# dlwns147/amq

Measured on AMD Instinct MI355X. Metric: decode tokens/s, Llama-2-7B AMQ mixed 2/3/4-bit avg-3-bit, batch 1, higher is better.
Workload: dtype f16; 1 GPU; Llama-2-7B shapes, synthesized avg-3.0-bit per-layer arch (bits_usage 2.982), batch 1 decode after a 64-token prefill, one stream per GPU; parallelism=replicas x1, prompt=64, group_size=128

## Files before the change

amq_amd/_lib.py:

```python
import ctypes
import os

_HERE = os.path.dirname(os.path.abspath(__file__))
LIB_PATH = os.path.join(_HERE, "libamq_hip.so")
AB_LIB_PATH = os.path.join(_HERE, "libamq_hip_ab.so")

AMQ_OK = 0
MODE_HQQ, MODE_FMA, MODE_FMA1 = 0, 1, 2
PRO_NONE, PRO_RMSNORM, PRO_SILU_MUL = 0, 1, 2
MAX_SEGMENTS = 4
MATH_DEFAULT, MATH_LINEAR, MATH_GROUPSCALE, MATH_EXACT = 0, 1, 2, 3
FEWROW_AUTO, FEWROW_TILE, FEWROW_STREAM = 0, 1, 2
ABI_VERSION = 521
LOOKUP_STATE_WORDS = 32
STEP_STATE_STRIDE = 272
GEMM_AUTO, GEMM_TILED, GEMM_SKINNY, GEMM_RING, GEMM_RING128, GEMM_WS, GEMM_DEQ = 0, 1, 2, 3, 4, 5, 6

_vp, _i, _f, _sz = ctypes.c_void_p, ctypes.c_int, ctypes.c_float, ctypes.c_size_t


class Segment(ctypes.Structure):
    _fields_ = [("qweight_native", _vp), ("meta_native", _vp), ("bias", _vp), ("residual", _vp),
                ("y", _vp), ("N", _i), ("bits", _i), ("mode", _i), ("y_stride", _i)]

# ... 32 lines not shown
    "amq_gemm_f16": (_i, [_i, _i, _vp, _vp, _vp, _vp, _vp, _i, _i, _i, _i, _i, _i, _vp]),
    "amq_linear_f16": (_i, [_i, _i, _vp, _vp, _vp, _vp, _vp, _i, _i, _i, _i, _vp]),
    "amq_gemm_splitk_workspace_bytes": (_sz, [_i, _i, _i]),
    "amq_gemm_splitk_f16": (_i, [_i, _i, _vp, _vp, _vp, _vp, _vp, _i, _i, _i, _i, _i, _i, _vp, _sz, _vp]),
    "amq_compat_workspace_bytes": (_sz, [_i, _i, _i, _i]),
    "amq_vecquantmatmul_faster_old": (_i, [_i, _vp, _vp, _vp, _vp, _vp, _i, _i, _i, _i, _i, _vp, _sz, _i, _vp]),
    "amq_gemv_4bit": (_i, [_vp, _vp, _vp, _vp, _vp, _i, _i, _i, _i, _vp, _sz, _i, _vp]),
    "amq_gemm_4bit": (_i, [_vp, _vp, _vp, _vp, _vp, _i, _i, _i, _i, _vp, _sz, _i, _vp]),
    "amq_rmsnorm_f16": (_i, [_vp, _vp, _vp, _i, _i, _f, _vp]),
    "amq_gemv_f16w": (_i, [_vp, _vp, _vp, _vp, _vp, _f, _i, _i, _vp]),
    "amq_attn_decode_f16": (_i, [_vp, _vp, _vp, _vp, _vp, _vp, _vp, _i, _i, _i, _i, _i, _i, _f, _vp, _vp]),
    "amq_rope_table_f16": (_i, [_vp, _i, _f, _vp]),
    "amq_rope_table_freqs_f16": (_i, [_vp, _i, _vp, _f, _vp]),
    "amq_decode_tail_f16": (_i, [_vp, _i, _vp, _i, _vp, _vp, _vp, _vp, _vp, _i, _vp]),
    "amq_attn_decode_cur_f16": (_i, [_vp, _vp, _vp, _vp, _vp, _vp, _vp, _i, _i, _i, _i, _i, _vp]),
    "amq_gemm_res_f16": (_i, [_i, _i, _vp, _vp, _vp, _vp, _vp, _vp, _i, _i, _i, _i, _i, _i, _vp, _sz, _vp]),
    "amq_xfrag_bytes": (_sz, [_i, _i]),
    "amq_xfrag_f16": (_i, [_vp, _vp, _i, _i, ctypes.c_longlong, ctypes.c_longlong, _vp]),
    "amq_rmsnorm_xfrag_f16": (_i, [_vp, _vp, _vp, _i, _i, _f, _vp]),
    "amq_gemm_xfrag_f16": (_i, [_i, _i, _vp, _vp, _vp, _vp, _vp, _vp, _vp, _i, _i, _i, _i, _i, _vp]),
    "amq_gemm_gated_fused": (_i, [_i, _i, _i, _i, _i]),
    "amq_gemm_gated_fused_g": (_i, [_i, _i, _i, _i, _i, _i]),
    "amq_gemm_gated_f16": (_i, [_i, _i, _i, _vp, _vp, _vp, _vp, _vp, _vp, _i, _i, _i, _i, _i, _vp, _sz, _vp]),
    "amq_attn_decode_split_workspace_bytes": (_sz, [_i, _i, _i]),
    "amq_attn_decode_split_f16": (_i, [_vp, _vp, _vp, _vp, _vp, _vp, _vp, _vp, _i, _i, _i, _i, _i, _i, _f, _vp, _i, _vp, _sz, _vp, _vp]),
    "amq_gemm_xfrag_grouped_f16": (_i, [ctypes.POINTER(Segment), _i, _vp, _i, _i, _i, _vp]),
    "amq_gemm_xfrag_grouped_form_f16": (_i, [ctypes.POINTER(Segment), _i, _vp, _i, _i, _i, _i, _i, _vp]),
    "amq_attn_prefill_xfrag_f16": (_i, [_vp, _vp, _vp, _vp, _i, _i, _i, _i, _i] + [ctypes.c_longlong] * 5 + [_vp]),
    "amq_gemv_f16w_rows": (_i, [_vp, _vp, _vp, _vp, _vp, _f, _i, _i, _i, _vp]),
    "amq_decode_tail_batch_f16": (_i, [_vp, _i, _vp, _i, _vp, _vp, _vp, _vp, _vp, _i, _i, _vp]),
    "amq_decode_tail_suppress_f16": (_i, [_vp, _i, _vp, _i, _vp, _vp, _vp, _vp, _vp, _i, _i, _vp, _vp]),
    "amq_sample_f16": (_i, [_vp, _i, _i, _vp, _vp, _vp, _vp, _vp, _i, _i, _vp]),
    "amq_decode_tail_sample_f16": (_i, [_vp, _i, _vp, _i, _vp, _vp, _vp, _vp, _vp, _i, _i, _vp, _vp, _vp]),
    "amq_set_token_f16": (_i, [_vp, _i, _vp, _i, _i, _vp, _vp, _vp, _vp, _vp, _i, _i, _vp]),
    "amq_attn_decode_seq_f16": (_i, [_vp, _vp, _vp, _vp, _vp, _vp, _vp, _i, _i, _i, _i, _i, _i, _vp, _sz, _vp, _vp]),
    "amq_decode_tail_seq_f16": (_i, [_vp, _i, _vp, _i, _vp, _vp, _vp, _vp, _i, _i, _vp, _vp]),
    "amq_decode_tail_sample_seq_f16": (_i, [_vp, _i, _vp, _i, _vp, _vp, _vp, _vp, _i, _i, _vp, _vp, _vp]),
    "amq_set_token_seq_f16": (_i, [_vp, _i, _vp, _i, _i, _vp, _vp, _vp, _vp, _i, _i, _vp]),
    "amq_attn_decode_rows_f16": (_i, [_vp, _vp, _vp, _vp, _vp, _vp, _vp, _i, _i, _i, _i, _i, _i, _vp, _sz, _vp, _vp]),
    "amq_decode_tail_lookup_f16": (_i, [_vp, _i, _vp, _i, _vp, _vp, _vp, _vp, _i, _i, _vp, _vp, _vp, _i, _vp]),
    "amq_attn_prefill_f16": (_i, [_vp, _vp, _vp, _vp, _i, _i, _i, _i, _i, _i] + [ctypes.c_longlong] * 10 + [_vp]),
    "amq_rope_cache_f16": (_i, [_vp, _vp, _vp, _vp, _vp, _vp, _i, _i, _i, _i, _i, _i, _i, _vp]),
    "amq_rope_cache_batch_f16": (_i, [_vp, _vp, _vp, _vp, _vp, _vp, _i, _i, _i, _i, _i, _i, _i, _i, _vp]),
    "amq_rope_rows_f16": (_i, [_vp, _vp, _vp, _i, _i, _i, _i, _i, _i, _i, _vp]),
    "amq_silu_mul_f16": (_i, [_vp, _vp, _vp, _sz, _vp]),
    "amq_gemv_grouped_f16": (_i, [ctypes.POINTER(Segment), _i, _vp, _vp, _vp, _f, _i, _i, _i, _i, _i, ctypes.POINTER(GemvOpts), _vp]),
    "amq_gemv_grouped_sums_f16": (_i, [ctypes.POINTER(Segment), _i, _vp, _vp, _f, _vp, _vp, _i, _i, _i, _vp]),
    "amq_gemm_f16w_f16": (_i, [_vp, _vp, _vp, _vp, _vp, _vp, _i, _i, _i, _i, _i, _vp]),
    "amq_gemm_route_workspace_bytes": (_sz, [_i, _i, _i, _i]),
    "amq_gemm_route_workspace_bytes_g": (_sz, [_i, _i, _i, _i, _i]),
# ... 135 lines not shown
```

amq_amd/csrc/amq_capi.hip:

```cpp
#include "../../include/amq_hip.h"
#ifdef AMQ_AB_ROUTES
#include "../../include/amq_hip_ab.h"
#endif
#include "amq_common.cuh"
#include "amq_kernels.h"

#include <stdarg.h>
#include <stdio.h>
#include <vector>

namespace {

thread_local char g_err[512] = "";

int fail(int code, const char* fmt, ...) {
    va_list ap;
    va_start(ap, fmt);
    vsnprintf(g_err, sizeof(g_err), fmt, ap);
    va_end(ap);
    return code;
}

int check_hip(hipError_t e, const char* what) {
    if (e == hipSuccess) return AMQ_OK;
// ... 695 lines not shown

int amq_attn_decode_cur_f16(const void* q, const void* k, const void* v, void* kcache, void* vcache, void* out,
                            const void* step_state, int batch, int n_heads, int n_kv_heads, int head_dim, int max_seq,
                            void* stream) {
    if (!q || !k || !v || !kcache || !vcache || !out || !step_state) return fail(AMQ_EINVAL, "null pointer");
    if (n_heads > 255) return fail(AMQ_ESHAPE, "at most 255 heads");
    if (head_dim != 128) return fail(AMQ_ESHAPE, "head_dim must be 128 (got %d)", head_dim);
    if (batch < 1 || n_heads < 1 || n_kv_heads < 1 || (n_heads % n_kv_heads) != 0)
        return fail(AMQ_ESHAPE, "bad head configuration (%d q heads, %d kv heads)", n_heads, n_kv_heads);
    if (max_seq < 1) return fail(AMQ_ESHAPE, "bad max_seq %d", max_seq);
    if (6 * 128 + (size_t)max_seq * 4 + 17 * 1024 > LDS_LIMIT) return fail(AMQ_ESHAPE, "max_seq=%d too long for the single-pass decode attention", max_seq);
    amq::AttnArgs a{q, k, v, kcache, vcache, out, nullptr, 0, n_heads, n_kv_heads, max_seq, 10000.0f, nullptr, step_state};
    return check_hip(amq::launch_attn_decode(a, batch, (hipStream_t)stream), "attn_decode_cur");
}

size_t amq_attn_decode_split_workspace_bytes(int batch, int n_heads, int n_splits) {
    if (batch < 1 || n_heads < 1 || n_splits < 1) return 0;
    return (size_t)batch * n_heads * n_splits * 132 * sizeof(float);
}

int amq_attn_decode_split_f16(const void* q, const void* k, const void* v, void* kcache, void* vcache, void* out,
                              const void* step_state, const int* pos_dev, int pos, int batch, int n_heads, int n_kv_heads,
                              int head_dim, int max_seq, float rope_theta, const void* rope_table, int n_splits,
                              void* workspace, size_t workspace_bytes, void* tickets, void* stream) {
    if (!q || !k || !v || !kcache || !vcache || !out || !workspace || !tickets) return fail(AMQ_EINVAL, "null pointer");
    if (head_dim != 128) return fail(AMQ_ESHAPE, "head_dim must be 128 (got %d)", head_dim);
    if (batch < 1 || batch > 65535 || n_heads < 1 || n_heads > 255 || n_kv_heads < 1 || (n_heads % n_kv_heads) != 0)
        return fail(AMQ_ESHAPE, "bad head configuration (batch %d, %d q heads, %d kv heads)", batch, n_heads, n_kv_heads);
    if (n_splits < 1 || n_splits > 1024) return fail(AMQ_EINVAL, "n_splits must be 1..1024 (got %d)", n_splits);
    if (max_seq < 1 || (!step_state && !pos_dev && (pos < 0 || pos >= max_seq)))
// ... 135 lines not shown
    if (max_seq < 1) return fail(AMQ_ESHAPE, "bad max_seq %d", max_seq);
    if (n_splits < 0 || n_splits > 1024) return fail(AMQ_EINVAL, "n_splits must be 0 (one workgroup per head) or 1..1024 (got %d)", n_splits);
    amq::AttnArgs a{q, k, v, kcache, vcache, out, nullptr, 0, n_heads, n_kv_heads, max_seq, 10000.0f, nullptr, step_states, true};
    if (n_splits == 0) {
        if (6 * 128 + (size_t)max_seq * 4 + 17 * 1024 > LDS_LIMIT) return fail(AMQ_ESHAPE, "max_seq=%d too long for the single-pass decode attention", max_seq);
        return check_hip(amq::launch_attn_decode(a, batch, (hipStream_t)stream), "attn_decode_seq");
    }
    if (!workspace || !tickets) return fail(AMQ_EINVAL, "null pointer (workspace / tickets are required with n_splits >= 1)");
    int chunk = (((max_seq + n_splits - 1) / n_splits) + 31) & ~31;
    chunk = chunk < amq::ATT_MIN_CHUNK ? amq::ATT_MIN_CHUNK : chunk;
    if (6 * 128 + (size_t)chunk * 4 + 17 * 1024 > LDS_LIMIT)
        return fail(AMQ_ESHAPE, "max_seq=%d over %d splits leaves chunks of %d keys: too long", max_seq, n_splits, chunk);
    const size_t need = amq_attn_decode_split_workspace_bytes(batch, n_heads, n_splits);
    if (workspace_bytes < need) return fail(AMQ_EINVAL, "workspace too small: need %zu bytes, got %zu", need, workspace_bytes);
    return check_hip(amq::launch_attn_decode_split(a, batch, n_splits, workspace, tickets, (hipStream_t)stream), "attn_decode_seq (split)");
}

static int tail_seq_check(const void* logits, int vocab, const void* embed, int hidden, const void* token, const void* step_states, const void* x,
                          const void* rope_table, int rope_rows, int batch) {
    if (!logits || !embed || !token || !step_states || !x || !rope_table) return fail(AMQ_EINVAL, "null pointer");
    if (rope_rows < 1) return fail(AMQ_EINVAL, "rope_rows must be the number of rows of rope_table");
    if (vocab < 1 || hidden < 8 || (hidden % 8) != 0) return fail(AMQ_ESHAPE, "need vocab >= 1 and hidden %% 8 == 0 (got %d, %d)", vocab, hidden);
    if (batch < 1 || batch > 65535) return fail(AMQ_ESHAPE, "bad batch %d", batch);
    return AMQ_OK;
}

int amq_decode_tail_seq_f16(const void* logits, int vocab, const void* embed, int hidden, long long* token, void* step_states, void* x,
                            const void* rope_table, int rope_rows, int batch, const int* suppress_ids, void* stream) {
    if (int rc = tail_seq_check(logits, vocab, embed, hidden, token, step_states, x, rope_table, rope_rows, batch)) return rc;
    if (batch > 1 && (vocab % 8) != 0) return fail(AMQ_ESHAPE, "batched rows need vocab %% 8 == 0 (16-byte aligned logits rows)");
// ... 80 lines not shown
```

amq_amd/csrc/amq_decode.hip:

```cpp
#include "amq_common.cuh"
#include "amq_kernels.h"

namespace amq {

__device__ __forceinline__ float wave_sum_f(float v) {
#pragma unroll
    for (int off = 32; off > 0; off >>= 1) v += __shfl_xor(v, off);
    return v;
}
__device__ __forceinline__ float wave_max_f(float v) {
#pragma unroll
    for (int off = 32; off > 0; off >>= 1) v = fmaxf(v, __shfl_xor(v, off));
    return v;
}

template <bool FRAG>
__global__ __launch_bounds__(256) void rmsnorm_kernel(const _Float16* x, const _Float16* gamma, _Float16* y, int M, int K, float eps) {
    __shared__ float red[4];
    const int m = blockIdx.x;
    const bool live = m < M;
    const _Float16* xr = x + (size_t)(live ? m : 0) * K;
    float ss = 0.f;
    for (int c = threadIdx.x; c < (K >> 3); c += 256) {
        h8 v = *(const h8*)(xr + 8 * c);
// ... 299 lines not shown
                       __builtin_bit_cast(float, __builtin_amdgcn_readlane(__builtin_bit_cast(int, v), 16))),
                 fmaxf(__builtin_bit_cast(float, __builtin_amdgcn_readlane(__builtin_bit_cast(int, v), 32)),
                       __builtin_bit_cast(float, __builtin_amdgcn_readlane(__builtin_bit_cast(int, v), 48))));
}

constexpr int ATT_THREADS = 512;
constexpr int ATT_GROUPS = ATT_THREADS / 16;
constexpr int ATT_PF = 12;
#ifndef AMQ_ATT_SPEC
#define AMQ_ATT_SPEC 2
#endif
constexpr int ATT_SPEC = AMQ_ATT_SPEC;

struct AttnRest {
    void* out; const void* rope_table; int pos; float rope_theta;
#ifdef AMQ_STAMP
    unsigned long long* stamps;
#endif
};
#ifdef AMQ_STAMP
extern unsigned long long* g_stamp_ptr;
#define ATT_STAMP(slot_) do { if (rest.stamps && threadIdx.x == 0) rest.stamps[(size_t)blockIdx.x * 16 + (slot_)] = __builtin_amdgcn_s_memrealtime(); } while (0)
#else
#define ATT_STAMP(slot_) do { } while (0)
#endif

constexpr int ATT_ROWS_MAX = 8;
constexpr int ATT_ROWS_LDS = 2 * (ATT_ROWS_MAX - 1) * ATT_D * 2;
template <bool SEQ, bool ROWS = false>
__global__ __launch_bounds__(ATT_THREADS) void attn_decode_kernel(void* p_kc, void* p_vc, const void* p_state, int p_heads,
                                                                   int p_max_seq, const void* p_q, const void* p_k,
                                                                   const void* p_v, AttnRest rest) {
    const void* const p_state0 = p_state;
    if (SEQ) p_state = (const char*)p_state + (size_t)blockIdx.y * STEP_STRIDE;
    extern __shared__ __attribute__((aligned(16))) unsigned char smem[];
    _Float16* qs = (_Float16*)smem;
    _Float16* ks = (_Float16*)smem + ATT_D;
    _Float16* vs = (_Float16*)smem + 2 * ATT_D;
    float* sc = (float*)(smem + 6 * ATT_D);
    __shared__ float red[2 * ATT_THREADS / 64];
    __shared__ float part[ATT_GROUPS][ATT_D];
    const int h = blockIdx.x, b = blockIdx.y, tid = threadIdx.x;
    const int cb = ROWS ? 0 : b;
    const int n_heads = p_heads & 0xFF, n_kv_heads = (p_heads >> 8) & 0xFF, max_seq = p_max_seq;
    const bool cur_mode = (p_heads >> 16) & 1;
    const void* p_cur = cur_mode ? p_state : nullptr;
    int pos;
    if (cur_mode) pos = *(const int*)((const char*)p_state + 256);
    else if (p_state) pos = *(const int*)p_state;
    else pos = rest.pos;
    const int group = n_heads / n_kv_heads;
    const int kvh = h / group;
    const int grp = tid >> 4, l16 = tid & 15;
    const _Float16* q = (const _Float16*)p_q + ((size_t)b * n_heads + h) * ATT_D;
    const _Float16* kn = (const _Float16*)p_k + ((size_t)b * n_kv_heads + kvh) * ATT_D;
    const _Float16* vn = (const _Float16*)p_v + ((size_t)b * n_kv_heads + kvh) * ATT_D;
    _Float16* kc = (_Float16*)p_kc + ((size_t)cb * n_kv_heads + kvh) * (size_t)max_seq * ATT_D;
    _Float16* vc = (_Float16*)p_vc + ((size_t)cb * n_kv_heads + kvh) * (size_t)max_seq * ATT_D;

    ATT_STAMP(0);
    _Float16 q0 = 0, q1 = 0, k0 = 0, k1 = 0, v0 = 0, v1 = 0;
    h2 cs_cur = {(_Float16)1.f, (_Float16)0.f}, cs_tab = {(_Float16)1.f, (_Float16)0.f};
    if (tid < 64) {
        q0 = q[tid]; q1 = q[tid + 64];
        k0 = kn[tid]; k1 = kn[tid + 64];
// ... 626 lines not shown

hipError_t launch_attn_decode_split(const AttnArgs& a, int batch, int n_splits, void* ws, void* tickets, hipStream_t st) {
    if (!a.rows && attn_decode_takes_gqa(a.n_heads, a.n_kv_heads, a.max_seq, n_splits)) return launch_attn_decode_gqa(a, batch, n_splits, ws, tickets, st);
    StreamDevice sd_(st);
    const size_t lds = 6 * ATT_D + (size_t)att_chunk_max(a.max_seq, n_splits) * 4;
#ifndef AMQ_ATT_RING_WIDE
#define AMQ_ATT_RING_WIDE 12
#endif
#ifndef AMQ_ATT_RING_NARROW
#define AMQ_ATT_RING_NARROW 4
#endif
    if ((long)a.n_heads * batch * n_splits <= 256) return launch_attn_decode_split_ring<AMQ_ATT_RING_WIDE>(a, batch, n_splits, ws, tickets, lds, st);
    return launch_attn_decode_split_ring<AMQ_ATT_RING_NARROW>(a, batch, n_splits, ws, tickets, lds, st);
}

hipError_t launch_attn_decode(const AttnArgs& a, int batch, hipStream_t st) {
    StreamDevice sd_(st);
    const size_t lds = a.rows ? ((6 * ATT_D + (size_t)a.max_seq * 4 + 15) & ~(size_t)15) + ATT_ROWS_LDS : 6 * ATT_D + (size_t)a.max_seq * 4;
    const auto kern = a.rows ? attn_decode_kernel<true, true> : a.seq ? attn_decode_kernel<true> : attn_decode_kernel<false>;
    if (lds > 64 * 1024) {
        hipError_t e = hipFuncSetAttribute((const void*)kern, hipFuncAttributeMaxDynamicSharedMemorySize, (int)lds);
        if (e != hipSuccess) return e;
    }
    AttnRest rest{a.out, a.rope_table, a.pos, a.rope_theta};
#ifdef AMQ_STAMP
    rest.stamps = g_stamp_ptr;
#endif
    const bool cur = a.rope_cur != nullptr;
    hipLaunchKernelGGL(kern, dim3(a.n_heads, batch), dim3(ATT_THREADS), lds, st, a.kcache, a.vcache,
                       cur ? a.rope_cur : (const void*)a.pos_dev, a.n_heads | (a.n_kv_heads << 8) | ((int)cur << 16), a.max_seq,
                       a.q, a.k, a.v, rest);
    return hipGetLastError();
}

}
```

amq_amd/csrc/amq_kernels.h:

```cpp
#pragma once
#include <hip/hip_runtime.h>
#include <stddef.h>
#include <stdint.h>

namespace amq {

inline hipError_t ensure_dyn_lds(unsigned long long& done_mask, const void* fn, int bytes) {
    int dev = 0;
    hipError_t e = hipGetDevice(&dev);
    if (e != hipSuccess) return e;
    const unsigned long long bit = 1ull << (dev & 63);
    if (__atomic_load_n(&done_mask, __ATOMIC_RELAXED) & bit) return hipSuccess;
    e = hipFuncSetAttribute(fn, hipFuncAttributeMaxDynamicSharedMemorySize, bytes);
    if (e == hipSuccess) __atomic_fetch_or(&done_mask, bit, __ATOMIC_RELAXED);
    return e;
}

struct StreamDevice {
    int prev = -1;
    bool switched = false;
    explicit StreamDevice(hipStream_t st) {
        hipDevice_t dev = 0;
        if (st == nullptr || hipGetDevice(&prev) != hipSuccess || hipStreamGetDevice(st, &dev) != hipSuccess) return;
        if ((int)dev != prev && hipSetDevice((int)dev) == hipSuccess) switched = true;
// ... 92 lines not shown
struct AttnArgs {
    const void* q;
    const void* k;
    const void* v;
    void* kcache;
    void* vcache;
    void* out;
    const int* pos_dev;
    int pos;
    int n_heads, n_kv_heads, max_seq;
    float rope_theta;
    const void* rope_table;
    const void* rope_cur;
    bool seq = false;
    bool rows = false;
};
constexpr int STEP_STRIDE = 272;
hipError_t launch_rope_table(void* tab, int max_seq, float theta, hipStream_t st);
hipError_t launch_rope_table_freqs(void* tab, int max_seq, const void* inv_freq, float scale, hipStream_t st);
hipError_t launch_attn_decode(const AttnArgs& a, int batch, hipStream_t st);
#ifndef AMQ_ATT_MIN_CHUNK
#define AMQ_ATT_MIN_CHUNK 256
#endif
constexpr int ATT_MIN_CHUNK = AMQ_ATT_MIN_CHUNK;
hipError_t launch_attn_decode_split(const AttnArgs& a, int batch, int n_splits, void* ws, void* tickets, hipStream_t st);
#ifndef AMQ_ATT_GQA
#define AMQ_ATT_GQA 1
#endif
bool attn_decode_takes_gqa(int n_heads, int n_kv_heads, int max_seq, int n_splits);
int attn_decode_gqa_iters(int max_seq, int n_splits);
hipError_t launch_attn_decode_gqa(const AttnArgs& a, int batch, int n_splits, void* ws, void* tickets, hipStream_t st);
// ... 106 lines not shown
```

amq_amd/llama.py:

```python
import math
from typing import NamedTuple

import torch

from . import ops
from .arch import MODEL_CONFIGS, arch_bits, rope_inv_freq, uniform_arch
from .hqq_format import HQQWeights

EPS = 1e-5
ROPE_THETA = 10000.0


class _Lin:
    __slots__ = ("qn", "mn", "bits", "mode", "N", "K", "bias")

    def __init__(self, qn, mn, bits, mode, N, K, bias=None):
        self.qn, self.mn, self.bits, self.mode, self.N, self.K, self.bias = qn, mn, bits, mode, N, K, bias

    def seg(self, y, residual=None):
        return dict(qn=self.qn, mn=self.mn, bits=self.bits, mode=self.mode, N=self.N, y=y, residual=residual, bias=self.bias)

    def nbytes(self):
        return self.qn.numel() * 4 + self.mn.numel() * 2 + (0 if self.bias is None else self.bias.numel() * 2)

# ... 106 lines not shown
        if self.held:
            self.runner.set_suppressed(self.before)
            self.held = False

    def __exit__(self, *exc):
        self.runner.set_suppressed(self.before)
        return False


class QuantLlama:
    ENGINE_MAX_SEQ = 512
    DOWN_FUSED_ROWS = 1
    NORM_FUSED_ROWS = 4
    NORM_SUMS = True
    FUSE_QKV_ATTN = False
    ENGINE_DEFAULT = False
    all_logits = False
    fine = False

    def __init__(self, config, arch_linear=None, device="cuda:0", max_seq=256, seed=0, synthetic=True,
                 hqq_layers=None, dense=None, batch=1, engine=None, prebuilt=None, group=128, rope=None, ragged=False, lookup=0, ngram_max=2):
        if isinstance(config, str):
            config = MODEL_CONFIGS[config]
        if not 1 <= int(batch) <= 8:
            raise ValueError("batch must be 1..8")
        self.B = int(batch)
        self.ragged = bool(ragged)
        self.lookup = int(lookup or 0)
        if self.lookup:
            if not 1 <= self.lookup <= ops.LOOKUP_MAX_ROWS - 1:
# ... 87 lines not shown
        self.xn = torch.zeros(R, self.H, **f16)
        self.q = torch.zeros(R, self.H, **f16)
        self.k = torch.zeros(R, self.kvd, **f16)
        self.v = torch.zeros(R, self.kvd, **f16)
        self.att = torch.zeros(R, self.H, **f16)
        self.gate = torch.zeros(R, self.I, **f16)
        self.up = torch.zeros(R, self.I, **f16)
        self._init_step_state(rope if rope is not None else rope_inv_freq(config))
        self.has_bias = any(blk[n].bias is not None for blk in self.blocks for n in config["linear"])
        self.plan = step_plan(R, self.H, self.I, self.fine, ops.gemv_max_rows(self.H, plain=True), ops.gemv_max_rows(self.I, plain=not self.fine),
                              ops.gemv_max_rows(self.I, plain=not self.fine, norm=False), self.NORM_SUMS, self.NORM_FUSED_ROWS, self.DOWN_FUSED_ROWS)
        self.ss = torch.zeros(R, self.H // 16, dtype=torch.float32, device=dev) if self.plan.norm == NORM_FROM_SUMS else None
        self.can_fuse_qkv_attn = (R == 1 and max_seq <= ops.ATTN_SPLIT_FROM and self.H <= 8192 and not self.fine and not self.has_bias
                                  and not self.ragged)
        self.fuse_qkv_attn = self.FUSE_QKV_ATTN and self.can_fuse_qkv_attn
        self._tickets = torch.zeros(max(self.nh, 64), dtype=torch.int32, device=dev)
        eligible = self.R == 1 and max_seq <= self.ENGINE_MAX_SEQ and self.H == self.nh * 128 and not self.fine and not self.has_bias and not self.ragged
        if engine and not eligible:
            raise ValueError("the decode engine needs batch 1 and max_seq <= %d" % self.ENGINE_MAX_SEQ)
        self.engine = None
        if engine is None:
            engine = self.ENGINE_DEFAULT
        if eligible and engine:
            self.engine = ops.DecodeEngine(
                [dict({n: dict(qn=blk[n].qn, mn=blk[n].mn, bits=blk[n].bits, mode=blk[n].mode, N=blk[n].N) for n in ops.ENGINE_LINEARS},
                      ln1=blk["ln1"], ln2=blk["ln2"], kc=blk["kc"], vc=blk["vc"]) for blk in self.blocks],
                self.H, self.I, self.nh, self.nkv, max_seq, self.eps, self.x.view(-1), self.rope_cur)

    def _init_step_state(self, rope):
        dev, R, max_seq = self.dev, self.R, self.max_seq
# ... 101 lines not shown
            raise ValueError("the fused q/k/v + attention launch keeps one position (batch 1): not offered with ragged=True")
        from_sums = plan.norm == NORM_FROM_SUMS
        first = plan.first_norm
        for blk in self.blocks:
            if self.fuse_qkv_attn:
                ops.gemv_qkv_attn(self.x, [blk["self_attn.q_proj"].seg(self.q.view(-1)), blk["self_attn.k_proj"].seg(self.k.view(-1)),
                                           blk["self_attn.v_proj"].seg(self.v.view(-1))], H, blk["ln1"], self.eps, blk["kc"], blk["vc"],
                                  self.att.view(-1), self.rope_cur, self.nh, self.nkv, self._tickets)
            else:
                self._behind_norm(first, blk["ln1"], [blk["self_attn.q_proj"].seg(self.q), blk["self_attn.k_proj"].seg(self.k),
                                                      blk["self_attn.v_proj"].seg(self.v)])
                if self.lookup:
                    ops.attn_decode_rows(self.q, self.k, self.v, blk["kc"], blk["vc"], self.att, self.rope_cur, self.pos, self.nh, self.nkv)
                else:
                    ops.attn_decode(self.q, self.k, self.v, blk["kc"], blk["vc"], self.att, self.pos, self.nh, self.nkv, self.theta,
                                    cur=self.rope_cur)
            o_proj, down = [blk["self_attn.o_proj"].seg(self.x, residual=self.x)], [blk["mlp.down_proj"].seg(self.x, residual=self.x)]
            if from_sums:
                ops.gemv_grouped_sums(self.att, o_proj, H, sums_out=self.ss)
            else:
                ops.gemv_grouped(self.att, o_proj, H)
            self._behind_norm(plan.norm, blk["ln2"], [blk["mlp.gate_proj"].seg(self.gate), blk["mlp.up_proj"].seg(self.up)])
            if plan.down == DOWN_FUSED:
                ops.gemv_grouped(self.gate, down, self.I, prologue=ops.PRO_SILU_MUL, x2=self.up)
            elif plan.down == DOWN_GEMV_SUMS:
                ops.gemv_grouped_sums(ops.silu_mul(self.gate, self.up, out=self.gate), down, self.I, sums_out=self.ss)
            elif plan.down == DOWN_GEMV:
                ops.gemv_grouped(ops.silu_mul(self.gate, self.up, out=self.gate), down, self.I)
            else:
                d = blk["mlp.down_proj"]
                ops.gemm(ops.silu_mul(self.gate, self.up, out=self.gate), d.qn, d.mn, d.bits, d.mode, d.N, d.K, bias=d.bias, residual=self.x, out=self.x)
            first = plan.block_norm
        ops.gemv_f16w(self.x.reshape(-1) if self.R == 1 else self.x, self.lm_head, gamma=self.norm, eps=self.eps, out=self.logits)
        self._tail(sampled)

    def _behind_norm(self, how, gamma, segments):
        if how == NORM_FROM_SUMS:
            ops.gemv_grouped_sums(self.x, segments, self.H, gamma=gamma, eps=self.eps, sums_in=self.ss)
        elif how == NORM_LAUNCH:
            ops.gemv_grouped(ops.rmsnorm(self.x, gamma, self.eps, out=self.xn), segments, self.H)
        else:
            ops.gemv_grouped(self.x, segments, self.H, prologue=ops.PRO_RMSNORM, gamma=gamma, eps=self.eps)

    def _tail(self, sampled):
        if self.lookup:
            if sampled:
                raise ValueError("lookup: speculative decoding here is greedy (the sampled tail draws one token per row)")
            ops.decode_tail_lookup(self.logits, self.embed, self.token, self.pos, self.x, self.lookup_state, self.history, self.rope_tab, self.rope_cur,
                                   suppress=self.suppress)
# ... 644 lines not shown
```

amq_amd/ops.py:

```python
import ctypes
import os

import torch

from . import _lib
from ._lib import (MODE_HQQ, MODE_FMA, MODE_FMA1, PRO_NONE, PRO_RMSNORM, PRO_SILU_MUL, Segment, GemvOpts, EngineBlock, EngineLinear,
                   GEMM_AUTO, GEMM_TILED, GEMM_SKINNY, GEMM_RING, GEMM_RING128, GEMM_WS, GEMM_DEQ, MATH_DEFAULT, MATH_EXACT, MATH_LINEAR, MATH_GROUPSCALE)

GROUP = 128


def _need(t, dtype, name, numel=None):
    if not isinstance(t, torch.Tensor) or not t.is_cuda:
        raise ValueError(f"{name}: expected a tensor on the GPU")
    if t.dtype != dtype:
        raise ValueError(f"{name}: expected {dtype}, got {t.dtype}")
    if not t.is_contiguous():
        raise ValueError(f"{name}: must be contiguous")
    if numel is not None and t.numel() != numel:
        raise ValueError(f"{name}: expected {numel} elements, got {t.numel()}")


FINE_GROUPS = (64, 32)

# ... 951 lines not shown
        if want > 32 and 32 * n_kv_heads * batch >= ATTN_CUS // 2:
            want = 32
        per = ATTN_GQA_KEYS or max(128 if max_seq <= 2048 else 256, -(-max_seq // want))
        per = -(-per // 128) * 128
        return max(2, -(-max_seq // per))
    s = max(1, round(max_seq / ATTN_CHUNK))
    wg = max(1, n_heads * batch)
    if ATTN_CUS % wg == 0:
        step = ATTN_CUS // wg
        s = max(step, round(s / step) * step) if s >= step else s
        while s >= step and (-(-max_seq // s) + 31) // 32 * 32 > ATTN_PREFETCH_KEYS:
            s += step
    return s


def attn_decode(q, k, v, kcache, vcache, out, pos, n_heads, n_kv_heads, rope_theta=10000.0, table=None, cur=None, n_splits=0):
    B = kcache.shape[0]
    max_seq = kcache.shape[2]
    if n_splits == 0:
        n_splits = attn_decode_splits(max_seq, n_heads, B, n_kv_heads)
    _need(q, torch.float16, "q", B * n_heads * 128)
    _need(k, torch.float16, "k", B * n_kv_heads * 128)
    _need(v, torch.float16, "v", B * n_kv_heads * 128)
    _need(kcache, torch.float16, "kcache", B * n_kv_heads * max_seq * 128)
    _need(vcache, torch.float16, "vcache", B * n_kv_heads * max_seq * 128)
    _need(out, torch.float16, "out", B * n_heads * 128)
    states, nseq = _seq_state(cur, pos)
    if states is not None:
        if nseq != B:
            raise ValueError(f"a step state of {nseq} sequences for caches of {B}")
        lib = _lib.load()
        if n_splits > 1:
            wsb = lib.amq_attn_decode_split_workspace_bytes(B, n_heads, n_splits)
            ws, tk = _ATTN_WS.get(q.device, wsb // 4), _ATTN_TICKETS.get(q.device, B * n_heads)
            _lib.check(lib.amq_attn_decode_seq_f16(_lib.ptr(q), _lib.ptr(k), _lib.ptr(v), _lib.ptr(kcache), _lib.ptr(vcache), _lib.ptr(out), states, B,
                                                   n_heads, n_kv_heads, 128, max_seq, n_splits, _lib.ptr(ws), wsb, _lib.ptr(tk), _lib.current_stream()))
        else:
            _lib.check(lib.amq_attn_decode_seq_f16(_lib.ptr(q), _lib.ptr(k), _lib.ptr(v), _lib.ptr(kcache), _lib.ptr(vcache), _lib.ptr(out), states, B,
                                                   n_heads, n_kv_heads, 128, max_seq, 0, None, 0, None, _lib.current_stream()))
        return out
    if isinstance(pos, torch.Tensor):
        _need(pos, torch.int32, "pos", 1)
        pos_dev, pos_i = ctypes.cast(pos.data_ptr(), ctypes.c_void_p), 0
    else:
        pos_dev, pos_i = None, int(pos)
        if not 0 <= pos_i < max_seq:
            raise ValueError(f"pos {pos_i} outside the cache (max_seq={max_seq})")
    if cur is not None:
        _need(cur, torch.float16, "rope_cur", 128)
        if pos_dev is None or pos.data_ptr() != cur.data_ptr() + 256:
            raise ValueError("cur / pos must be the two views of one step-state block (ops.new_step_state)")
    if table is not None:
        _need(table, torch.float16, "rope table", max_seq * 128)
    if n_splits > 1:
        lib = _lib.load()
        wsb = lib.amq_attn_decode_split_workspace_bytes(B, n_heads, n_splits)
        ws = _ATTN_WS.get(q.device, wsb // 4)
        tk = _ATTN_TICKETS.get(q.device, B * n_heads)
        _lib.check(lib.amq_attn_decode_split_f16(_lib.ptr(q), _lib.ptr(k), _lib.ptr(v), _lib.ptr(kcache), _lib.ptr(vcache),
                                                 _lib.ptr(out), _lib.ptr(cur), pos_dev, pos_i, B, n_heads, n_kv_heads, 128,
                                                 max_seq, ctypes.c_float(rope_theta), _lib.ptr(table), n_splits,
                                                 _lib.ptr(ws), wsb, _lib.ptr(tk), _lib.current_stream()))
        return out
    if cur is not None:
        _lib.check(_lib.load().amq_attn_decode_cur_f16(_lib.ptr(q), _lib.ptr(k), _lib.ptr(v), _lib.ptr(kcache), _lib.ptr(vcache),
                                                       _lib.ptr(out), _lib.ptr(cur), B, n_heads, n_kv_heads, 128, max_seq,
                                                       _lib.current_stream()))
        return out
    _lib.check(_lib.load().amq_attn_decode_f16(_lib.ptr(q), _lib.ptr(k), _lib.ptr(v), _lib.ptr(kcache), _lib.ptr(vcache),
                                               _lib.ptr(out), pos_dev, pos_i, B, n_heads, n_kv_heads, 128, max_seq,
                                               ctypes.c_float(rope_theta), _lib.ptr(table), _lib.current_stream()))
    return out


LOOKUP_STATE_WORDS = _lib.LOOKUP_STATE_WORDS
LOOKUP_DRAFTS, LOOKUP_NGRAM, LOOKUP_MODE, LOOKUP_COUNT, LOOKUP_STEPS, LOOKUP_ACCEPTED, LOOKUP_TICKET, LOOKUP_DRAFT, LOOKUP_ARGMAX = 0, 1, 2, 3, 4, 5, 6, 8, 16
LOOKUP_MAX_ROWS = 8

# ... 88 lines not shown
```

include/amq_hip.h:

```cpp
#ifndef AMQ_HIP_H
#define AMQ_HIP_H

#include <stddef.h>
#include <stdint.h>

#ifdef __cplusplus
extern "C" {
#endif

#define AMQ_VERSION 521

#define AMQ_OK            0
#define AMQ_EINVAL       -1
#define AMQ_ESHAPE       -2
#define AMQ_ELAUNCH      -3
#define AMQ_EUNSUPPORTED -4

#define AMQ_MODE_HQQ 0
#define AMQ_MODE_FMA 1
#define AMQ_MODE_FMA1 2

#define AMQ_PRO_NONE     0
#define AMQ_PRO_RMSNORM  1
#define AMQ_PRO_SILU_MUL 2
// ... 91 lines not shown
int amq_rmsnorm_f16(const void* x, const void* gamma, void* y, int M, int K, float eps, void* stream);
int amq_gemv_f16w(const void* x, const void* W, const void* bias, void* y, const void* gamma, float eps,
                  int N, int K, void* stream);
int amq_gemv_f16w_rows(const void* x, const void* W, const void* bias, void* y, const void* gamma, float eps, int M,
                       int N, int K, void* stream);
int amq_attn_decode_f16(const void* q, const void* k, const void* v, void* kcache, void* vcache, void* out,
                        const int* pos_dev, int pos, int batch, int n_heads, int n_kv_heads, int head_dim,
                        int max_seq, float rope_theta, const void* rope_table, void* stream);
int amq_rope_table_f16(void* table, int max_seq, float rope_theta, void* stream);
int amq_rope_table_freqs_f16(void* table, int max_seq, const float* inv_freq, float scale, void* stream);

int amq_attn_decode_cur_f16(const void* q, const void* k, const void* v, void* kcache, void* vcache, void* out,
                            const void* step_state, int batch, int n_heads, int n_kv_heads, int head_dim, int max_seq,
                            void* stream);

size_t amq_attn_decode_split_workspace_bytes(int batch, int n_heads, int n_splits);
int amq_attn_decode_split_f16(const void* q, const void* k, const void* v, void* kcache, void* vcache, void* out,
                              const void* step_state, const int* pos_dev, int pos, int batch, int n_heads, int n_kv_heads,
                              int head_dim, int max_seq, float rope_theta, const void* rope_table, int n_splits,
                              void* workspace, size_t workspace_bytes, void* tickets, void* stream);

int amq_decode_tail_f16(const void* logits, int vocab, const void* embed, int hidden, long long* token, int* pos, void* x,
                        const void* rope_table, void* rope_cur, int rope_rows, void* stream);
int amq_set_token_f16(const long long* token_in, int n_in, const void* embed, int vocab, int hidden, long long* token, const int* pos, void* x,
                      const void* rope_table, void* rope_cur, int rope_rows, int batch, void* stream);
int amq_decode_tail_suppress_f16(const void* logits, int vocab, const void* embed, int hidden, long long* token, int* pos, void* x,
                                 const void* rope_table, void* rope_cur, int rope_rows, int batch, const int* suppress_ids, void* stream);
int amq_decode_tail_batch_f16(const void* logits, int vocab, const void* embed, int hidden, long long* token, int* pos, void* x,
                              const void* rope_table, void* rope_cur, int rope_rows, int batch, void* stream);

#define AMQ_SAMPLE_ADVANCE 1
#define AMQ_SAMPLE_EOS 2
int amq_sample_f16(const void* logits, int rows, int vocab, void* state, const int* suppress_ids, const float* u_in, long long* token_out,
                   unsigned char* kept_out, int seq0, int flags, void* stream);
int amq_decode_tail_sample_f16(const void* logits, int vocab, const void* embed, int hidden, long long* token, int* pos, void* x,
                               const void* rope_table, void* rope_cur, int rope_rows, int batch, const int* suppress_ids, void* state,
                               void* stream);

#define AMQ_STEP_STATE_STRIDE 272
int amq_attn_decode_seq_f16(const void* q, const void* k, const void* v, void* kcache, void* vcache, void* out, void* step_states, int batch,
                            int n_heads, int n_kv_heads, int head_dim, int max_seq, int n_splits, void* workspace, size_t workspace_bytes,
                            void* tickets, void* stream);
int amq_decode_tail_seq_f16(const void* logits, int vocab, const void* embed, int hidden, long long* token, void* step_states, void* x,
                            const void* rope_table, int rope_rows, int batch, const int* suppress_ids, void* stream);
int amq_decode_tail_sample_seq_f16(const void* logits, int vocab, const void* embed, int hidden, long long* token, void* step_states, void* x,
                                   const void* rope_table, int rope_rows, int batch, const int* suppress_ids, void* state, void* stream);
int amq_set_token_seq_f16(const long long* token_in, int n_in, const void* embed, int vocab, int hidden, long long* token, void* step_states, void* x,
                          const void* rope_table, int rope_rows, int batch, void* stream);

#define AMQ_LOOKUP_MAX_ROWS 8
int amq_attn_decode_rows_f16(const void* q, const void* k, const void* v, void* kcache, void* vcache, void* out, void* step_states, int rows,
                             int n_heads, int n_kv_heads, int head_dim, int max_seq, int n_splits, void* workspace, size_t workspace_bytes,
                             void* tickets, void* stream);
#define AMQ_LOOKUP_STATE_WORDS 32
int amq_decode_tail_lookup_f16(const void* logits, int vocab, const void* embed, int hidden, long long* token, void* step_states, void* x,
                               const void* rope_table, int rope_rows, int rows, const int* suppress_ids, void* lookup_state, int* history,
                               int history_cap, void* stream);
// ... 63 lines not shown
```

Before: 756.6 tokens/s.

## Prefetch o_proj weights into cache with extra workgroups in decode attention

Adds extra workgroups to the single-pass decode attention launch that stream the upcoming o_proj packed weights through the cache while the attention heads run. The reads are spread across workgroups, optionally following the row-tile layout so each workgroup touches the tiles its later GEMV counterpart would read. The aim is to hide the o_proj GEMV's DRAM latency behind the otherwise underused attention kernel. In exchange the prefetch competes for bandwidth and CUs with attention and only pays off if the lines are still in L2/MALL when o_proj runs.

```diff
diff --git a/amq_amd/_lib.py b/amq_amd/_lib.py
--- a/amq_amd/_lib.py
+++ b/amq_amd/_lib.py
@@ -70,6 +70,9 @@
     "amq_rope_table_freqs_f16": (_i, [_vp, _i, _vp, _f, _vp]),
     "amq_decode_tail_f16": (_i, [_vp, _i, _vp, _i, _vp, _vp, _vp, _vp, _vp, _i, _vp]),
     "amq_attn_decode_cur_f16": (_i, [_vp, _vp, _vp, _vp, _vp, _vp, _vp, _i, _i, _i, _i, _i, _vp]),
+    "amq_attn_decode_warm_f16": (_i, [_vp, _vp, _vp, _vp, _vp, _vp, _vp, _i, _i, _i, _i, _i, _vp, _vp, ctypes.c_longlong, ctypes.c_longlong]),
+    "amq_attn_warm_workgroups": (_i, []),
+    "amq_attn_warm_ranges": (_i, [_i, ctypes.c_longlong, ctypes.c_longlong, _i, ctypes.POINTER(ctypes.c_longlong), _i]),
     "amq_gemm_res_f16": (_i, [_i, _i, _vp, _vp, _vp, _vp, _vp, _vp, _i, _i, _i, _i, _i, _i, _vp, _sz, _vp]),
     "amq_xfrag_bytes": (_sz, [_i, _i]),
     "amq_xfrag_f16": (_i, [_vp, _vp, _i, _i, ctypes.c_longlong, ctypes.c_longlong, _vp]),
@@ -90,6 +93,7 @@
     "amq_decode_tail_sample_f16": (_i, [_vp, _i, _vp, _i, _vp, _vp, _vp, _vp, _vp, _i, _i, _vp, _vp, _vp]),
     "amq_set_token_f16": (_i, [_vp, _i, _vp, _i, _i, _vp, _vp, _vp, _vp, _vp, _i, _i, _vp]),
     "amq_attn_decode_seq_f16": (_i, [_vp, _vp, _vp, _vp, _vp, _vp, _vp, _i, _i, _i, _i, _i, _i, _vp, _sz, _vp, _vp]),
+    "amq_attn_decode_warm_seq_f16": (_i, [_vp, _vp, _vp, _vp, _vp, _vp, _vp, _i, _i, _i, _i, _i, _i, _vp, _sz, _vp, _vp, _vp, ctypes.c_longlong, ctypes.c_longlong]),
     "amq_decode_tail_seq_f16": (_i, [_vp, _i, _vp, _i, _vp, _vp, _vp, _vp, _i, _i, _vp, _vp]),
     "amq_decode_tail_sample_seq_f16": (_i, [_vp, _i, _vp, _i, _vp, _vp, _vp, _vp, _i, _i, _vp, _vp, _vp]),
     "amq_set_token_seq_f16": (_i, [_vp, _i, _vp, _i, _i, _vp, _vp, _vp, _vp, _i, _i, _vp]),
diff --git a/amq_amd/csrc/amq_capi.hip b/amq_amd/csrc/amq_capi.hip
--- a/amq_amd/csrc/amq_capi.hip
+++ b/amq_amd/csrc/amq_capi.hip
@@ -733,6 +733,40 @@
     return check_hip(amq::launch_attn_decode(a, batch, (hipStream_t)stream), "attn_decode_cur");
 }
 
+static int attn_warm_check(const void* warm, long long warm_bytes, long long warm_rt_bytes) {
+    if (warm_bytes < 0) return fail(AMQ_EINVAL, "warm_bytes must be >= 0 (got %lld)", warm_bytes);
+    if (warm_bytes > amq::ATT_WARM_MAX_BYTES) return fail(AMQ_EINVAL, "warm_bytes %lld beyond %lld", warm_bytes, amq::ATT_WARM_MAX_BYTES);
+    if (((uintptr_t)warm & 15) != 0) return fail(AMQ_EINVAL, "warm must be 16-byte aligned");
+    if (warm_rt_bytes < 0 || (warm_rt_bytes & 15) != 0) return fail(AMQ_EINVAL, "warm_rt_bytes must be 0 (linear slices) or a positive multiple of 16 (got %lld)", warm_rt_bytes);
+    return AMQ_OK;
+}
+
+int amq_attn_decode_warm_f16(const void* q, const void* k, const void* v, void* kcache, void* vcache, void* out,
+                             const void* step_state, int batch, int n_heads, int n_kv_heads, int head_dim, int max_seq,
+                             void* stream, const void* warm, long long warm_bytes, long long warm_rt_bytes) {
+    if (!q || !k || !v || !kcache || !vcache || !out || !step_state) return fail(AMQ_EINVAL, "null pointer");
+    if (n_heads > 255) return fail(AMQ_ESHAPE, "at most 255 heads");
+    if (head_dim != 128) return fail(AMQ_ESHAPE, "head_dim must be 128 (got %d)", head_dim);
+    if (batch < 1 || n_heads < 1 || n_kv_heads < 1 || (n_heads % n_kv_heads) != 0)
+        return fail(AMQ_ESHAPE, "bad head configuration (%d q heads, %d kv heads)", n_heads, n_kv_heads);
+    if (max_seq < 1) return fail(AMQ_ESHAPE, "bad max_seq %d", max_seq);
+    if (6 * 128 + (size_t)max_seq * 4 + 17 * 1024 > LDS_LIMIT) return fail(AMQ_ESHAPE, "max_seq=%d too long for the single-pass decode attention", max_seq);
+    if (int rc = attn_warm_check(warm, warm_bytes, warm_rt_bytes)) return rc;
+    amq::AttnArgs a{q, k, v, kcache, vcache, out, nullptr, 0, n_heads, n_kv_heads, max_seq, 10000.0f, nullptr, step_state};
+    a.warm = warm; a.warm_bytes = warm_bytes; a.warm_rt_bytes = warm_rt_bytes;
+    return check_hip(amq::launch_attn_decode(a, batch, (hipStream_t)stream), "attn_decode_warm");
+}
+
+int amq_attn_warm_ranges(int w, long long warm_bytes, long long warm_rt_bytes, int n_heads, long long* ranges, int cap) {
+    if (warm_bytes < 0 || warm_bytes > amq::ATT_WARM_MAX_BYTES || warm_rt_bytes < 0 || (warm_rt_bytes & 15) != 0 || cap < 0 || (cap > 0 && !ranges)) {
+        fail(AMQ_EINVAL, "bad arguments");
+        return -1;
+    }
+    return amq::attn_warm_ranges(w, amq::ATT_WARM_WGS, warm_bytes, warm_rt_bytes, n_heads, ranges, cap);
+}
+
+int amq_attn_warm_workgroups(void) { return amq::ATT_WARM_WGS; }
+
 size_t amq_attn_decode_split_workspace_bytes(int batch, int n_heads, int n_splits) {
     if (batch < 1 || n_heads < 1 || n_splits < 1) return 0;
     return (size_t)batch * n_heads * n_splits * 132 * sizeof(float);
@@ -898,6 +932,24 @@
     const size_t need = amq_attn_decode_split_workspace_bytes(batch, n_heads, n_splits);
     if (workspace_bytes < need) return fail(AMQ_EINVAL, "workspace too small: need %zu bytes, got %zu", need, workspace_bytes);
     return check_hip(amq::launch_attn_decode_split(a, batch, n_splits, workspace, tickets, (hipStream_t)stream), "attn_decode_seq (split)");
+}
+
+int amq_attn_decode_warm_seq_f16(const void* q, const void* k, const void* v, void* kcache, void* vcache, void* out, void* step_states, int batch,
+                                 int n_heads, int n_kv_heads, int head_dim, int max_seq, int n_splits, void* workspace, size_t workspace_bytes,
+                                 void* tickets, void* stream, const void* warm, long long warm_bytes, long long warm_rt_bytes) {
+    if (int rc = attn_warm_check(warm, warm_bytes, warm_rt_bytes)) return rc;
+    if (n_splits != 0) return amq_attn_decode_seq_f16(q, k, v, kcache, vcache, out, step_states, batch, n_heads, n_kv_heads, head_dim, max_seq, n_splits,
+                                                      workspace, workspace_bytes, tickets, stream);
+    if (!q || !k || !v || !kcache || !vcache || !out || !step_states) return fail(AMQ_EINVAL, "null pointer");
+    if (head_dim != 128) return fail(AMQ_ESHAPE, "head_dim must be 128 (got %d)", head_dim);
+    if (batch < 1 || batch > 65535 || n_heads < 1 || n_heads > 255 || n_kv_heads < 1 || (n_heads % n_kv_heads) != 0)
+        return fail(AMQ_ESHAPE, "bad head configuration (batch %d, %d q heads, %d kv heads)", batch, n_heads, n_kv_heads);
+    if (max_seq < 1) return fail(AMQ_ESHAPE, "bad max_seq %d", max_seq);
+    if (6 * 128 + (size_t)max_seq * 4 + 17 * 1024 > LDS_LIMIT) return fail(AMQ_ESHAPE, "max_seq=%d too long for the single-pass decode attention", max_seq);
+    if (int rc = attn_warm_check(warm, warm_bytes, warm_rt_bytes)) return rc;
+    amq::AttnArgs a{q, k, v, kcache, vcache, out, nullptr, 0, n_heads, n_kv_heads, max_seq, 10000.0f, nullptr, step_states, true};
+    a.warm = warm; a.warm_bytes = warm_bytes; a.warm_rt_bytes = warm_rt_bytes;
+    return check_hip(amq::launch_attn_decode(a, batch, (hipStream_t)stream), "attn_decode_warm_seq");
 }
 
 static int tail_seq_check(const void* logits, int vocab, const void* embed, int hidden, const void* token, const void* step_states, const void* x,
diff --git a/amq_amd/csrc/amq_decode.hip b/amq_amd/csrc/amq_decode.hip
--- a/amq_amd/csrc/amq_decode.hip
+++ b/amq_amd/csrc/amq_decode.hip
@@ -337,6 +337,7 @@
 
 struct AttnRest {
     void* out; const void* rope_table; int pos; float rope_theta;
+    const void* warm; long long warm_bytes, warm_rt_bytes; int warm_wgs;
 #ifdef AMQ_STAMP
     unsigned long long* stamps;
 #endif
@@ -347,6 +348,27 @@
 #else
 #define ATT_STAMP(slot_) do { } while (0)
 #endif
+
+constexpr int ATT_WARM_FLIGHT = 4;
+__device__ __forceinline__ void attn_warm_loop(const void* warm, long long bytes, long long rt_bytes, int W, int heads, int w, int tid) {
+    const AttnWarmSlice s = attn_warm_slice(w, W, bytes, rt_bytes, heads);
+    const unsigned long long limit = (unsigned long long)bytes & ~15ULL;
+    const char* base = (const char*)warm;
+    unsigned seen = 0;
+    for (unsigned c = s.c0 + tid; c < s.c1; c += ATT_WARM_FLIGHT * ATT_THREADS) {
+        u4 v[ATT_WARM_FLIGHT];
+#pragma unroll
+        for (int j = 0; j < ATT_WARM_FLIGHT; ++j) {
+            const unsigned cj = c + j * ATT_THREADS;
+            const unsigned long long off = attn_warm_chunk_byte(s, cj < s.c1 ? cj : s.c0, rt_bytes);
+            v[j] = (u4){0u, 0u, 0u, 0u};
+            if (cj < s.c1 && off + 16 <= limit) v[j] = *(const u4*)(base + off);
+        }
+#pragma unroll
+        for (int j = 0; j < ATT_WARM_FLIGHT; ++j) seen |= v[j].x | v[j].y | v[j].z | v[j].w;
+    }
+    if (seen & 1) __builtin_amdgcn_endpgm();
+}
 
 constexpr int ATT_ROWS_MAX = 8;
 constexpr int ATT_ROWS_LDS = 2 * (ATT_ROWS_MAX - 1) * ATT_D * 2;
@@ -372,6 +394,12 @@
     if (cur_mode) pos = *(const int*)((const char*)p_state + 256);
     else if (p_state) pos = *(const int*)p_state;
     else pos = rest.pos;
+    if constexpr (!ROWS) {
+        if ((int)blockIdx.x >= (p_heads & 0xFF)) {
+            if (blockIdx.y == 0) attn_warm_loop(rest.warm, rest.warm_bytes, rest.warm_rt_bytes, rest.warm_wgs, p_heads & 0xFF, (int)blockIdx.x - (p_heads & 0xFF), threadIdx.x);
+            return;
+        }
+    }
     const int group = n_heads / n_kv_heads;
     const int kvh = h / group;
     const int grp = tid >> 4, l16 = tid & 15;
@@ -1028,6 +1056,24 @@
     return launch_attn_decode_split_ring<AMQ_ATT_RING_NARROW>(a, batch, n_splits, ws, tickets, lds, st);
 }
 
+int attn_warm_ranges(int w, int W, long long bytes, long long rt_bytes, int heads, long long* out, int cap) {
+    const AttnWarmSlice s = attn_warm_slice(w, W, bytes, rt_bytes, heads);
+    const unsigned long long limit = (unsigned long long)bytes & ~15ULL;
+    int n = 0;
+    for (unsigned c = s.c0; c < s.c1;) {
+        const unsigned e = s.ct ? (c / s.ct + 1) * s.ct < s.c1 ? (c / s.ct + 1) * s.ct : s.c1 : s.c1;
+        const unsigned long long b0 = attn_warm_chunk_byte(s, c, rt_bytes);
+        unsigned long long b1 = b0 + ((unsigned long long)(e - c) << 4);
+        if (b1 > limit) b1 = limit;
+        if (b0 < b1) {
+            if (n < cap) { out[2 * n] = (long long)b0; out[2 * n + 1] = (long long)b1; }
+            ++n;
+        }
+        c = e;
+    }
+    return n;
+}
+
 hipError_t launch_attn_decode(const AttnArgs& a, int batch, hipStream_t st) {
     StreamDevice sd_(st);
     const size_t lds = a.rows ? ((6 * ATT_D + (size_t)a.max_seq * 4 + 15) & ~(size_t)15) + ATT_ROWS_LDS : 6 * ATT_D + (size_t)a.max_seq * 4;
@@ -1036,12 +1082,18 @@
         hipError_t e = hipFuncSetAttribute((const void*)kern, hipFuncAttributeMaxDynamicSharedMemorySize, (int)lds);
         if (e != hipSuccess) return e;
     }
-    AttnRest rest{a.out, a.rope_table, a.pos, a.rope_theta};
+    const bool warm = !a.rows && a.warm && (a.warm_bytes & ~15LL) != 0 && ATT_WARM_WGS > 0;
+#ifdef AMQ_ATT_WARM_LINEAR
+    const long long warm_rt = 0;
+#else
+    const long long warm_rt = a.warm_rt_bytes;
+#endif
+    AttnRest rest{a.out, a.rope_table, a.pos, a.rope_theta, warm ? a.warm : nullptr, warm ? a.warm_bytes : 0, warm ? warm_rt : 0, warm ? ATT_WARM_WGS : 0};
 #ifdef AMQ_STAMP
     rest.stamps = g_stamp_ptr;
 #endif
     const bool cur = a.rope_cur != nullptr;
-    hipLaunchKernelGGL(kern, dim3(a.n_heads, batch), dim3(ATT_THREADS), lds, st, a.kcache, a.vcache,
+    hipLaunchKernelGGL(kern, dim3(a.n_heads + (warm ? ATT_WARM_WGS : 0), batch), dim3(ATT_THREADS), lds, st, a.kcache, a.vcache,
                        cur ? a.rope_cur : (const void*)a.pos_dev, a.n_heads | (a.n_kv_heads << 8) | ((int)cur << 16), a.max_seq,
                        a.q, a.k, a.v, rest);
     return hipGetLastError();
diff --git a/amq_amd/csrc/amq_kernels.h b/amq_amd/csrc/amq_kernels.h
--- a/amq_amd/csrc/amq_kernels.h
+++ b/amq_amd/csrc/amq_kernels.h
@@ -130,7 +130,49 @@
     const void* rope_cur;
     bool seq = false;
     bool rows = false;
-};
+    const void* warm = nullptr;
+    long long warm_bytes = 0;
+    long long warm_rt_bytes = 0;
+};
+#ifndef AMQ_ATT_WARM_WGS
+#define AMQ_ATT_WARM_WGS 224
+#endif
+constexpr int ATT_WARM_WGS = AMQ_ATT_WARM_WGS;
+constexpr long long ATT_WARM_MAX_BYTES = 16LL << 30;
+struct AttnWarmSlice {
+    unsigned c0, c1;
+    unsigned ct;
+    unsigned r;
+};
+#if defined(__HIPCC__)
+#define AMQ_HD __host__ __device__
+#else
+#define AMQ_HD
+#endif
+AMQ_HD inline AttnWarmSlice attn_warm_slice(int w, int W, long long bytes, long long rt_bytes, int heads) {
+    const unsigned n = (unsigned)(((unsigned long long)bytes & ~15ULL) >> 4);
+    AttnWarmSlice s{0, 0, 0, 0};
+    if (w < 0 || w >= W || n == 0) return s;
+    unsigned total = n, parts = (unsigned)W, rank = (unsigned)w;
+    if (rt_bytes != 0) {
+        s.ct = (unsigned)(rt_bytes >> 4);
+        s.r = (unsigned)(heads + w) & 7u;
+        const unsigned tiles = n / s.ct + (n % s.ct != 0);
+        total = (tiles > s.r ? (tiles - s.r + 7) / 8 : 0) * s.ct;
+        parts = ((unsigned)W - 1 - ((unsigned)w & 7u)) / 8 + 1;
+        rank = (unsigned)w >> 3;
+    }
+    const unsigned base = total / parts, rem = total - base * parts;
+    s.c0 = rank * base + (rank < rem ? rank : rem);
+    s.c1 = s.c0 + base + (rank < rem ? 1 : 0);
+    return s;
+}
+AMQ_HD inline unsigned long long attn_warm_chunk_byte(const AttnWarmSlice& s, unsigned c, long long rt_bytes) {
+    if (s.ct == 0) return (unsigned long long)c << 4;
+    const unsigned q = c / s.ct, o = c - q * s.ct;
+    return ((unsigned long long)q * 8 + s.r) * (unsigned long long)rt_bytes + ((unsigned long long)o << 4);
+}
+int attn_warm_ranges(int w, int W, long long bytes, long long rt_bytes, int heads, long long* out, int cap);
 constexpr int STEP_STRIDE = 272;
 hipError_t launch_rope_table(void* tab, int max_seq, float theta, hipStream_t st);
 hipError_t launch_rope_table_freqs(void* tab, int max_seq, const void* inv_freq, float scale, hipStream_t st);
diff --git a/amq_amd/llama.py b/amq_amd/llama.py
--- a/amq_amd/llama.py
+++ b/amq_amd/llama.py
@@ -144,6 +144,7 @@
     NORM_FUSED_ROWS = 4
     NORM_SUMS = True
     FUSE_QKV_ATTN = False
+    ATTN_WARM = True
     ENGINE_DEFAULT = False
     all_logits = False
     fine = False
@@ -261,6 +262,7 @@
         self.can_fuse_qkv_attn = (R == 1 and max_seq <= ops.ATTN_SPLIT_FROM and self.H <= 8192 and not self.fine and not self.has_bias
                                   and not self.ragged)
         self.fuse_qkv_attn = self.FUSE_QKV_ATTN and self.can_fuse_qkv_attn
+        self.attn_warm = bool(self.ATTN_WARM and R == 1 and self.B == 1 and not self.lookup and max_seq <= ops.ATTN_SPLIT_FROM and not self.fine)
         self._tickets = torch.zeros(max(self.nh, 64), dtype=torch.int32, device=dev)
         eligible = self.R == 1 and max_seq <= self.ENGINE_MAX_SEQ and self.H == self.nh * 128 and not self.fine and not self.has_bias and not self.ragged
         if engine and not eligible:
@@ -392,7 +394,7 @@
                     ops.attn_decode_rows(self.q, self.k, self.v, blk["kc"], blk["vc"], self.att, self.rope_cur, self.pos, self.nh, self.nkv)
                 else:
                     ops.attn_decode(self.q, self.k, self.v, blk["kc"], blk["vc"], self.att, self.pos, self.nh, self.nkv, self.theta,
-                                    cur=self.rope_cur)
+                                    cur=self.rope_cur, warm=self._warm_of(blk["self_attn.o_proj"]) if self.attn_warm else None)
             o_proj, down = [blk["self_attn.o_proj"].seg(self.x, residual=self.x)], [blk["mlp.down_proj"].seg(self.x, residual=self.x)]
             if from_sums:
                 ops.gemv_grouped_sums(self.att, o_proj, H, sums_out=self.ss)
@@ -411,6 +413,11 @@
             first = plan.block_norm
         ops.gemv_f16w(self.x.reshape(-1) if self.R == 1 else self.x, self.lm_head, gamma=self.norm, eps=self.eps, out=self.logits)
         self._tail(sampled)
+
+    @staticmethod
+    def _warm_of(lin):
+        n_rt = lin.N // 16
+        return lin.qn, (16 * lin.K * lin.bits // 8 if n_rt <= 256 and lin.N % 16 == 0 else 0)
 
     def _behind_norm(self, how, gamma, segments):
         if how == NORM_FROM_SUMS:
diff --git a/amq_amd/ops.py b/amq_amd/ops.py
--- a/amq_amd/ops.py
+++ b/amq_amd/ops.py
@@ -989,7 +989,27 @@
     return s
 
 
-def attn_decode(q, k, v, kcache, vcache, out, pos, n_heads, n_kv_heads, rope_theta=10000.0, table=None, cur=None, n_splits=0):
+def attn_warm_ranges(w, nbytes, row_tile_bytes, n_heads):
+    lib = _lib.load()
+    cap = 64
+    while True:
+        buf = (ctypes.c_longlong * (2 * cap))()
+        n = lib.amq_attn_warm_ranges(int(w), int(nbytes), int(row_tile_bytes), int(n_heads), buf, cap)
+        if n < 0:
+            raise _lib.AmqError(f"libamq_hip error: {lib.amq_last_error().decode('utf-8', 'replace')}")
+        if n <= cap:
+            return [(buf[2 * i], buf[2 * i + 1]) for i in range(n)]
+        cap = n
+
+
+def _warm_args(warm, device):
+    t, rt = warm
+    if not (isinstance(t, torch.Tensor) and t.is_cuda and t.device == device and t.is_contiguous()):
+        raise ValueError("warm: a contiguous tensor on the launch's device")
+    return _lib.ptr(t), t.numel() * t.element_size(), int(rt)
+
+
+def attn_decode(q, k, v, kcache, vcache, out, pos, n_heads, n_kv_heads, rope_theta=10000.0, table=None, cur=None, n_splits=0, warm=None):
     B = kcache.shape[0]
     max_seq = kcache.shape[2]
     if n_splits == 0:
@@ -1010,6 +1030,10 @@
             ws, tk = _ATTN_WS.get(q.device, wsb // 4), _ATTN_TICKETS.get(q.device, B * n_heads)
             _lib.check(lib.amq_attn_decode_seq_f16(_lib.ptr(q), _lib.ptr(k), _lib.ptr(v), _lib.ptr(kcache), _lib.ptr(vcache), _lib.ptr(out), states, B,
                                                    n_heads, n_kv_heads, 128, max_seq, n_splits, _lib.ptr(ws), wsb, _lib.ptr(tk), _lib.current_stream()))
+        elif warm is not None:
+            wp, wb, wrt = _warm_args(warm, q.device)
+            _lib.check(lib.amq_attn_decode_warm_seq_f16(_lib.ptr(q), _lib.ptr(k), _lib.ptr(v), _lib.ptr(kcache), _lib.ptr(vcache), _lib.ptr(out), states, B,
+                                                        n_heads, n_kv_heads, 128, max_seq, 0, None, 0, None, _lib.current_stream(), wp, wb, wrt))
         else:
             _lib.check(lib.amq_attn_decode_seq_f16(_lib.ptr(q), _lib.ptr(k), _lib.ptr(v), _lib.ptr(kcache), _lib.ptr(vcache), _lib.ptr(out), states, B,
                                                    n_heads, n_kv_heads, 128, max_seq, 0, None, 0, None, _lib.current_stream()))
@@ -1037,6 +1061,14 @@
                                                  max_seq, ctypes.c_float(rope_theta), _lib.ptr(table), n_splits,
                                                  _lib.ptr(ws), wsb, _lib.ptr(tk), _lib.current_stream()))
         return out
+    if warm is not None and cur is None:
+        raise ValueError("warm: offered by the step-state forms (cur=) of the single-workgroup kernel")
+    if warm is not None:
+        wp, wb, wrt = _warm_args(warm, q.device)
+        _lib.check(_lib.load().amq_attn_decode_warm_f16(_lib.ptr(q), _lib.ptr(k), _lib.ptr(v), _lib.ptr(kcache), _lib.ptr(vcache),
+                                                        _lib.ptr(out), _lib.ptr(cur), B, n_heads, n_kv_heads, 128, max_seq,
+                                                        _lib.current_stream(), wp, wb, wrt))
+        return out
     if cur is not None:
         _lib.check(_lib.load().amq_attn_decode_cur_f16(_lib.ptr(q), _lib.ptr(k), _lib.ptr(v), _lib.ptr(kcache), _lib.ptr(vcache),
                                                        _lib.ptr(out), _lib.ptr(cur), B, n_heads, n_kv_heads, 128, max_seq,
diff --git a/include/amq_hip.h b/include/amq_hip.h
--- a/include/amq_hip.h
+++ b/include/amq_hip.h
@@ -129,6 +129,12 @@
                             const void* step_state, int batch, int n_heads, int n_kv_heads, int head_dim, int max_seq,
                             void* stream);
 
+int amq_attn_decode_warm_f16(const void* q, const void* k, const void* v, void* kcache, void* vcache, void* out,
+                             const void* step_state, int batch, int n_heads, int n_kv_heads, int head_dim, int max_seq,
+                             void* stream, const void* warm, long long warm_bytes, long long warm_rt_bytes);
+int amq_attn_warm_workgroups(void);
+int amq_attn_warm_ranges(int w, long long warm_bytes, long long warm_rt_bytes, int n_heads, long long* ranges, int cap);
+
 size_t amq_attn_decode_split_workspace_bytes(int batch, int n_heads, int n_splits);
 int amq_attn_decode_split_f16(const void* q, const void* k, const void* v, void* kcache, void* vcache, void* out,
                               const void* step_state, const int* pos_dev, int pos, int batch, int n_heads, int n_kv_heads,
@@ -156,6 +162,9 @@
 int amq_attn_decode_seq_f16(const void* q, const void* k, const void* v, void* kcache, void* vcache, void* out, void* step_states, int batch,
                             int n_heads, int n_kv_heads, int head_dim, int max_seq, int n_splits, void* workspace, size_t workspace_bytes,
                             void* tickets, void* stream);
+int amq_attn_decode_warm_seq_f16(const void* q, const void* k, const void* v, void* kcache, void* vcache, void* out, void* step_states, int batch,
+                                 int n_heads, int n_kv_heads, int head_dim, int max_seq, int n_splits, void* workspace, size_t workspace_bytes,
+                                 void* tickets, void* stream, const void* warm, long long warm_bytes, long long warm_rt_bytes);
 int amq_decode_tail_seq_f16(const void* logits, int vocab, const void* embed, int hidden, long long* token, void* step_states, void* x,
                             const void* rope_table, int rope_rows, int batch, const int* suppress_ids, void* stream);
 int amq_decode_tail_sample_seq_f16(const void* logits, int vocab, const void* embed, int hidden, long long* token, void* step_states, void* x,
```

After: 756.5 tokens/s, median of 2. Within noise of the previous version (-0.0%).
